# fujii-team/deComP

Measured on AMD Instinct MI355X. Metric: nmf_mu_iterations_per_s, higher is better.
Workload: dtype f32

## Files before the change

decomp_amd/csrc/gemm_mfma_bf16x6.hpp:

```cpp
#pragma once
#include "gemm_mfma_f32.hpp"

namespace dcp {

typedef __bf16 x6_bf16x4 __attribute__((ext_vector_type(4)));
typedef __bf16 x6_bf16x8 __attribute__((ext_vector_type(8)));

template <int BM_, int BN_, int WM_, int WN_, int MINW_>
struct X6Cfg {
    static constexpr int BM = BM_, BN = BN_, BK = 16, WM = WM_, WN = WN_, MINW = MINW_;
    static constexpr int NWAVES = (BM_ / WM_) * (BN_ / WN_);
    static constexpr int NTHREADS = 64 * NWAVES;
};
typedef X6Cfg<256, 256, 64, 64, 1> X6Huge;
typedef X6Cfg<128, 128, 64, 64, 2> X6Large;

template <int ROWS>
struct X6Panel {
    static constexpr int PLANE_BYTES = ROWS * 32;
    static constexpr int BYTES = 3 * PLANE_BYTES;
};

__device__ __forceinline__ int x6_chunk(int r, int q) { return r * 32 + ((q ^ ((r >> 3) & 1)) << 4); }

__device__ __forceinline__ void x6_split(f32x4 a, x6_bf16x4& h, x6_bf16x4& m, x6_bf16x4& l) {
    h = __builtin_convertvector(a, x6_bf16x4);
    const f32x4 r1 = a - __builtin_convertvector(h, f32x4);
    m = __builtin_convertvector(r1, x6_bf16x4);
    const f32x4 r2 = r1 - __builtin_convertvector(m, f32x4);
    l = __builtin_convertvector(r2, x6_bf16x4);
}

template <int LAY, int ROWS, int NT, int G>
__device__ __forceinline__ void x6_gload(f32x4 (&r)[G], const float* __restrict__ p, long ld, int row0, int k0,
                                         int tid) {
    static_assert(G * NT * 4 == ROWS * 16, "panel must be a whole number of 4-value groups per thread");
#pragma unroll
    for (int i = 0; i < G; ++i) {
        const int idx = tid + i * NT;
        if (LAY == KMAJOR) {
            const int row = idx >> 2, kq = idx & 3;
            r[i] = *reinterpret_cast<const f32x4*>(p + (long)(row0 + row) * ld + (k0 + 4 * kq));
        } else {
            const int g = idx % (ROWS / 4), k = idx / (ROWS / 4);
            r[i] = *reinterpret_cast<const f32x4*>(p + (long)(k0 + k) * ld + (row0 + 4 * g));
        }
    }
}

template <int ROWS>
__device__ __forceinline__ int x6_granule(int k, int g) {
    static_assert(ROWS >= 128, "the XOR swizzle needs 32 granules per k row");
    return k * (ROWS * 2) + ((g ^ ((k & 3) << 3)) << 3);
}

template <int LAY, int ROWS, int NT, int G>
__device__ __forceinline__ void x6_lds_store(char* s, const f32x4 (&r)[G], int tid) {
#pragma unroll
    for (int i = 0; i < G; ++i) {
        const int idx = tid + i * NT;
        int off;
        if (LAY == KMAJOR) {
            const int row = idx >> 2, kq = idx & 3;
            off = x6_chunk(row, kq >> 1) + ((kq & 1) << 3);
        } else {
            off = x6_granule<ROWS>(idx / (ROWS / 4), idx % (ROWS / 4));
        }
        x6_bf16x4 h, m, l;
        x6_split(r[i], h, m, l);
        *reinterpret_cast<x6_bf16x4*>(s + off) = h;
        *reinterpret_cast<x6_bf16x4*>(s + X6Panel<ROWS>::PLANE_BYTES + off) = m;
        *reinterpret_cast<x6_bf16x4*>(s + 2 * X6Panel<ROWS>::PLANE_BYTES + off) = l;
    }
}

template <int LAY, int ROWS>
__device__ __forceinline__ int x6_frag_off(int r0, int lane) {
    const int l31 = lane & 31, h = lane >> 5;
    if (LAY == KMAJOR) return x6_chunk(r0 + l31, h);
    const int q = (lane >> 2) & 3, pq = lane & 3, gh = (lane >> 4) & 1;
    return x6_granule<ROWS>(8 * h + q, (r0 >> 2) + 4 * gh + pq);
}

template <int LAY, int ROWS>
__device__ __forceinline__ x6_bf16x8 x6_frag(const char* plane, int off) {
    if (LAY == KMAJOR) return *reinterpret_cast<const x6_bf16x8*>(plane + off);
    typedef short s16x4 __attribute__((ext_vector_type(4)));
    typedef __attribute__((address_space(3))) s16x4 lds_s16x4;
    const s16x4 lo = __builtin_amdgcn_ds_read_tr16_b64_v4i16((lds_s16x4*)(plane + off));
    const s16x4 hi = __builtin_amdgcn_ds_read_tr16_b64_v4i16((lds_s16x4*)(plane + off + 4 * ROWS * 2));
    return __builtin_bit_cast(x6_bf16x8, __builtin_shufflevector(lo, hi, 0, 1, 2, 3, 4, 5, 6, 7));
}

template <class Cfg, int ALAY, int BLAY, class Epi>
__global__ void __launch_bounds__(Cfg::NTHREADS, Cfg::MINW) gemm_bf16x6_kernel(GemmProblem p, Epi epi) {
    constexpr int BM = Cfg::BM, BN = Cfg::BN, BK = Cfg::BK, WM = Cfg::WM, WN = Cfg::WN;
    constexpr int TM = WM / 32, TN = WN / 32;
    constexpr int WAVES_N = BN / WN;
    constexpr int NT = Cfg::NTHREADS;
    constexpr int GA = BM * BK / 4 / NT, GB = BN * BK / 4 / NT;
    constexpr int PA = X6Panel<BM>::PLANE_BYTES, PB = X6Panel<BN>::PLANE_BYTES;
    constexpr int BUF = X6Panel<BM>::BYTES + X6Panel<BN>::BYTES;
    static_assert(epi_mode<Epi>::value == 0 && !epi_rowbits<Epi>::value, "bf16x6 core: plain real epilogues");

    extern __shared__ __attribute__((aligned(16))) char x6_smem[];

    const int tid = threadIdx.x;
    const int lane = tid & 63, wave = tid >> 6;
    const int wm = wave / WAVES_N, wn = wave % WAVES_N;
    const int l31 = lane & 31, h = lane >> 5;

    const int lid = xcd_remap(blockIdx.x, gridDim.x);
    const int tiles = p.tiles_m * p.tiles_n;
    const int split = lid / tiles;
    const int t = lid - split * tiles;
    int mt, nt;
    if (p.mt_fast) {
        mt = t % p.tiles_m;
        nt = t / p.tiles_m;
    } else {
        nt = t % p.tiles_n;
        mt = t / p.tiles_n;
    }
    const int m0 = mt * BM;
    const int kbeg = split * p.klen;
    const int kend = min(p.K, kbeg + p.klen);
    const float* Bp = p.B;
    long ldb = p.ldb;
    int nB0 = nt * BN;
    int n0 = nB0;
    if (nt >= p.tiles_n1) {
        Bp = p.B2;
        ldb = p.ldb2;
        nB0 = (nt - p.tiles_n1) * BN;
        n0 = p.n_b1 + nB0;
    }

    f32x16 acc[TM][TN];
#pragma unroll
    for (int i = 0; i < TM; ++i)
#pragma unroll
        for (int j = 0; j < TN; ++j)
#pragma unroll
            for (int r = 0; r < 16; ++r) acc[i][j][r] = 0.0f;

    f32x4 ra[GA], rb[GB];
    const int nkb = (kend - kbeg) / BK;
    if (nkb > 0) {
        x6_gload<ALAY, BM, NT>(ra, p.A, p.lda, m0, kbeg, tid);
        x6_gload<BLAY, BN, NT>(rb, Bp, ldb, nB0, kbeg, tid);
        x6_lds_store<ALAY, BM, NT>(x6_smem, ra, tid);
        x6_lds_store<BLAY, BN, NT>(x6_smem + X6Panel<BM>::BYTES, rb, tid);
    }
    __syncthreads();

    int aoff[TM], boff[TN];
#pragma unroll
    for (int i = 0; i < TM; ++i) aoff[i] = x6_frag_off<ALAY, BM>(wm * WM + i * 32, lane);
#pragma unroll
    for (int j = 0; j < TN; ++j) boff[j] = x6_frag_off<BLAY, BN>(wn * WN + j * 32, lane);

    for (int kb = 0; kb < nkb; ++kb) {
        const int cur = kb & 1;
        const char* sA = x6_smem + cur * BUF;
        const char* sB = sA + X6Panel<BM>::BYTES;
        const bool more = (kb + 1) < nkb;
        if (more) {
            const int k0 = kbeg + (kb + 1) * BK;
            x6_gload<ALAY, BM, NT>(ra, p.A, p.lda, m0, k0, tid);
            x6_gload<BLAY, BN, NT>(rb, Bp, ldb, nB0, k0, tid);
        }
        x6_bf16x8 fb[3][TN];
#pragma unroll
        for (int pl = 0; pl < 3; ++pl)
#pragma unroll
            for (int j = 0; j < TN; ++j) fb[pl][j] = x6_frag<BLAY, BN>(sB + pl * PB, boff[j]);
        constexpr int TA[6] = {2, 0, 1, 1, 0, 0};
        constexpr int TB[6] = {0, 2, 1, 0, 1, 0};
#pragma unroll
        for (int i = 0; i < TM; ++i) {
            x6_bf16x8 fa[3];
#pragma unroll
            for (int pl = 0; pl < 3; ++pl) fa[pl] = x6_frag<ALAY, BM>(sA + pl * PA, aoff[i]);
#pragma unroll
            for (int tt = 0; tt < 6; ++tt)
#pragma unroll
                for (int j = 0; j < TN; ++j)
                    acc[i][j] = __builtin_amdgcn_mfma_f32_32x32x16_bf16(fa[TA[tt]], fb[TB[tt]][j], acc[i][j], 0, 0, 0);
            __builtin_amdgcn_sched_barrier(0);
        }
        if (more) {
            char* nxt = x6_smem + (cur ^ 1) * BUF;
            x6_lds_store<ALAY, BM, NT>(nxt, ra, tid);
            x6_lds_store<BLAY, BN, NT>(nxt + X6Panel<BM>::BYTES, rb, tid);
        }
        __syncthreads();
    }

    if constexpr (epi_vec4<Epi>::value) {
        const int tq = l31 & 3, col0 = (l31 & ~3);
#pragma unroll
        for (int i = 0; i < TM; ++i)
#pragma unroll
            for (int j = 0; j < TN; ++j)
#pragma unroll
                for (int g = 0; g < 4; ++g) {
                    f32x4 x;
#pragma unroll
                    for (int e = 0; e < 4; ++e) x[e] = acc[i][j][4 * g + e];
                    const f32x4 y = quad_transpose(x, tq);
                    epi.vec4(m0 + wm * WM + i * 32 + 8 * g + 4 * h + tq, n0 + wn * WN + j * 32 + col0, y, split);
                }
    } else {
#pragma unroll
        for (int i = 0; i < TM; ++i)
#pragma unroll
            for (int j = 0; j < TN; ++j) {
                const int col = n0 + wn * WN + j * 32 + l31;
#pragma unroll
                for (int r = 0; r < 16; ++r) {
                    const int row = m0 + wm * WM + i * 32 + (r & 3) + 8 * (r >> 2) + 4 * h;
                    epi(row, col, acc[i][j][r], split);
                }
            }
    }
}

template <class Epi>
inline bool x6_epi_ok(const Epi& epi) {
    if constexpr (epi_vec4<Epi>::value) return epi.vec_ok();
    else return true;
}

template <class Cfg>
inline bool x6_eligible(const GemmProblem& p) {
    auto al16 = [](const void* q) { return (reinterpret_cast<uintptr_t>(q) & 15) == 0; };
    const int n1 = p.B2 != nullptr ? p.n_b1 : p.N;
    bool ok = p.M > 0 && p.N > 0 && p.K > 0 && (p.M % Cfg::BM) == 0 && (n1 % Cfg::BN) == 0 &&
              ((p.N - n1) % Cfg::BN) == 0 && (p.K % 16) == 0 && p.A2 == nullptr && (p.lda % 4) == 0 &&
              (p.ldb % 4) == 0 && al16(p.A) && al16(p.B);
    if (p.B2 != nullptr) ok = ok && (p.ldb2 % 4) == 0 && al16(p.B2);
    if (p.ksplits > 1) ok = ok && (p.klen % 16) == 0 && p.klen > 0;
    return ok;
}

template <class Cfg, int ALAY, int BLAY, class Epi>
inline hipError_t launch_gemm_bf16x6(hipStream_t stream, GemmProblem p, const Epi& epi) {
    if (!x6_eligible<Cfg>(p) || !x6_epi_ok(epi)) return hipErrorInvalidValue;
    if (p.B2 == nullptr) p.n_b1 = p.N;
    p.m_a1 = p.M;
    p.tiles_m1 = p.tiles_m = p.M / Cfg::BM;
    p.tiles_n1 = p.n_b1 / Cfg::BN;
    p.tiles_n = p.tiles_n1 + (p.N - p.n_b1) / Cfg::BN;
    if (p.ksplits < 1) p.ksplits = 1;
    if (p.ksplits == 1) p.klen = p.K;
    p.vec_epi = epi_vec4<Epi>::value ? 1 : 0;
    p.al_mask = 0;
    const int grid = p.tiles_m * p.tiles_n * p.ksplits;
    if (grid <= 0) return hipSuccess;
    constexpr int lds_bytes = 2 * (X6Panel<Cfg::BM>::BYTES + X6Panel<Cfg::BN>::BYTES);
    const void* fn = reinterpret_cast<const void*>(&gemm_bf16x6_kernel<Cfg, ALAY, BLAY, Epi>);
    if constexpr (lds_bytes > 65536) {
        static DynLdsRaised raised;
        std::atomic<bool>& done = raised.on_current_device();
        if (!done) {
            hipError_t e = hipFuncSetAttribute(fn, hipFuncAttributeMaxDynamicSharedMemorySize, lds_bytes);
            if (e != hipSuccess) return e;
            done = true;
        }
    }
    hipLaunchKernelGGL((gemm_bf16x6_kernel<Cfg, ALAY, BLAY, Epi>), dim3(grid), dim3(Cfg::NTHREADS), lds_bytes,
                       stream, p, epi);
    return hipGetLastError();
}

}
```

Baseline: 661.8.

## Deepen bf16x6 GEMM prefetch and interleave LDS staging between MFMA groups

The K-loop now prefetches global data two blocks ahead instead of one. The LDS store and next global load for the A panel are placed in the middle of the first A-row group's MFMAs, and those for the B panel in the middle of the second group's. The last k-block is peeled and skips staging. The goal is to hide LDS write and global-load latency behind matrix instructions instead of storing after all MFMAs, at the cost of more complex scheduling. It also issues redundant clamped loads at the tail.

After: 678.9, median of 6. 2.6% higher.

```diff
diff --git a/decomp_amd/csrc/gemm_mfma_bf16x6.hpp b/decomp_amd/csrc/gemm_mfma_bf16x6.hpp
--- a/decomp_amd/csrc/gemm_mfma_bf16x6.hpp
+++ b/decomp_amd/csrc/gemm_mfma_bf16x6.hpp
@@ -1,5 +1,6 @@
 #pragma once
 #include "gemm_mfma_f32.hpp"
+#include <type_traits>
 
 namespace dcp {
 
@@ -144,6 +145,7 @@
 #pragma unroll
             for (int r = 0; r < 16; ++r) acc[i][j][r] = 0.0f;
 
+    static_assert(TM == 2, "one panel's staging per 32-row A block");
     f32x4 ra[GA], rb[GB];
     const int nkb = (kend - kbeg) / BK;
     if (nkb > 0) {
@@ -151,6 +153,9 @@
         x6_gload<BLAY, BN, NT>(rb, Bp, ldb, nB0, kbeg, tid);
         x6_lds_store<ALAY, BM, NT>(x6_smem, ra, tid);
         x6_lds_store<BLAY, BN, NT>(x6_smem + X6Panel<BM>::BYTES, rb, tid);
+        const int k1 = kbeg + min(1, nkb - 1) * BK;
+        x6_gload<ALAY, BM, NT>(ra, p.A, p.lda, m0, k1, tid);
+        x6_gload<BLAY, BN, NT>(rb, Bp, ldb, nB0, k1, tid);
     }
     __syncthreads();
 
@@ -160,16 +165,14 @@
 #pragma unroll
     for (int j = 0; j < TN; ++j) boff[j] = x6_frag_off<BLAY, BN>(wn * WN + j * 32, lane);
 
-    for (int kb = 0; kb < nkb; ++kb) {
+    constexpr int STAGE_AFTER = 2;
+    auto kblock = [&](int kb, auto stage_tag) {
+        constexpr bool STAGE = decltype(stage_tag)::value;
         const int cur = kb & 1;
         const char* sA = x6_smem + cur * BUF;
         const char* sB = sA + X6Panel<BM>::BYTES;
-        const bool more = (kb + 1) < nkb;
-        if (more) {
-            const int k0 = kbeg + (kb + 1) * BK;
-            x6_gload<ALAY, BM, NT>(ra, p.A, p.lda, m0, k0, tid);
-            x6_gload<BLAY, BN, NT>(rb, Bp, ldb, nB0, k0, tid);
-        }
+        char* nxt = x6_smem + (cur ^ 1) * BUF;
+        const int k2 = kbeg + min(kb + 2, nkb - 1) * BK;
         x6_bf16x8 fb[3][TN];
 #pragma unroll
         for (int pl = 0; pl < 3; ++pl)
@@ -177,25 +180,44 @@
             for (int j = 0; j < TN; ++j) fb[pl][j] = x6_frag<BLAY, BN>(sB + pl * PB, boff[j]);
         constexpr int TA[6] = {2, 0, 1, 1, 0, 0};
         constexpr int TB[6] = {0, 2, 1, 0, 1, 0};
-#pragma unroll
-        for (int i = 0; i < TM; ++i) {
+        auto group = [&](auto i_tag) {
+            constexpr int i = decltype(i_tag)::value;
             x6_bf16x8 fa[3];
 #pragma unroll
             for (int pl = 0; pl < 3; ++pl) fa[pl] = x6_frag<ALAY, BM>(sA + pl * PA, aoff[i]);
-#pragma unroll
-            for (int tt = 0; tt < 6; ++tt)
-#pragma unroll
-                for (int j = 0; j < TN; ++j)
-                    acc[i][j] = __builtin_amdgcn_mfma_f32_32x32x16_bf16(fa[TA[tt]], fb[TB[tt]][j], acc[i][j], 0, 0, 0);
+            auto mfmas = [&](int t0, int t1) {
+#pragma unroll
+                for (int tt = t0; tt < t1; ++tt)
+#pragma unroll
+                    for (int j = 0; j < TN; ++j)
+                        acc[i][j] =
+                            __builtin_amdgcn_mfma_f32_32x32x16_bf16(fa[TA[tt]], fb[TB[tt]][j], acc[i][j], 0, 0, 0);
+            };
+            if constexpr (STAGE) {
+                mfmas(0, STAGE_AFTER);
+                __builtin_amdgcn_sched_barrier(0);
+                if constexpr (i == 0) {
+                    x6_lds_store<ALAY, BM, NT>(nxt, ra, tid);
+                    x6_gload<ALAY, BM, NT>(ra, p.A, p.lda, m0, k2, tid);
+                } else {
+                    x6_lds_store<BLAY, BN, NT>(nxt + X6Panel<BM>::BYTES, rb, tid);
+                    x6_gload<BLAY, BN, NT>(rb, Bp, ldb, nB0, k2, tid);
+                }
+                __builtin_amdgcn_sched_barrier(0);
+                mfmas(STAGE_AFTER, 6);
+            } else {
+                mfmas(0, 6);
+            }
             __builtin_amdgcn_sched_barrier(0);
-        }
-        if (more) {
-            char* nxt = x6_smem + (cur ^ 1) * BUF;
-            x6_lds_store<ALAY, BM, NT>(nxt, ra, tid);
-            x6_lds_store<BLAY, BN, NT>(nxt + X6Panel<BM>::BYTES, rb, tid);
-        }
+        };
+        group(std::integral_constant<int, 0>{});
+        group(std::integral_constant<int, 1>{});
+    };
+    for (int kb = 0; kb + 1 < nkb; ++kb) {
+        kblock(kb, std::true_type{});
         __syncthreads();
     }
+    if (nkb > 0) kblock(nkb - 1, std::false_type{});
 
     if constexpr (epi_vec4<Epi>::value) {
         const int tq = l31 & 3, col0 = (l31 & ~3);
```
